# aghasemzadeh/OpenMPL

Hardware: AMD Instinct MI355X
Metric: poses/sec (V=4, J=17, batch=1024 per GPU) fp32 (higher is better)
Workload: dtype f32; 1 GPU; Human3.6M config: V=4 J=17 batch=1024 fp32, CHOSEN flag set, depth 12, DIM 32, heads 8; global_batch=1024, parallelism=single GPU

## Files before the change

### openmpl_amd/csrc/spt_packed.hip

```cpp
#include "spt_pack.hpp"
#include "spt_stage.hpp"

namespace mpl {

constexpr int ATS = 36;
constexpr int HS = 68;
constexpr int KV_F = SJ * SH * SEQ * 4;
constexpr int SPT3_RING_BYTES = (ROWS * XS + 2 * KV_F + ROWS * ATS) * 4;
constexpr int SPT3_LDS_BYTES = 160 * 1024;
constexpr int SPT3_HID_OFF = 3072;
constexpr int SPT3_Q_OFF = 20480;
static_assert(SPT3_HID_OFF + ROWS * HS <= 2 * KV_F + ROWS * ATS, "HID does not fit its alias");
static_assert((SPT3_HID_OFF + ROWS * HS - 2 * KV_F) * 4 <= SPT3_Q_OFF, "HID reaches into the staged qkv weights");
static_assert(SPT3_Q_OFF + 12 * 1024 <= ROWS * ATS * 4, "staged qkv weights do not fit behind HID in ATT");
static_assert(SPT3_RING_BYTES + 8 * 1024 + 2 * SPT3_NPAR * 4 <= SPT3_LDS_BYTES, "spare LDS too small");

typedef float f32x2 __attribute__((ext_vector_type(2)));

__device__ inline float spt_window_scale(float v) {
    if (!(v > 0.f) || !(v < 3.0e38f)) return 1.0f;
    int e;
    (void)frexpf(32768.0f / v, &e);
    e = e - 1 < -100 ? -100 : (e - 1 > 100 ? 100 : e - 1);
    return ldexpf(1.0f, e);
}

__global__ __launch_bounds__(256) void spt_pack_kernel(const float* __restrict__ qkv_w, const float* __restrict__ qkv_b,
                                                        const float* __restrict__ ln1_w, const float* __restrict__ ln1_b,
                                                        const float* __restrict__ proj_w, const float* __restrict__ proj_b,
                                                        const float* __restrict__ fc1_w, const float* __restrict__ fc1_b,
                                                        const float* __restrict__ ln2_w, const float* __restrict__ ln2_b,
                                                        const float* __restrict__ fc2_w, const float* __restrict__ fc2_b,
                                                        char* __restrict__ dst, int fold_q) {
    __shared__ float Wf[8192];
    __shared__ float cn[SPT_NCOL], sw[SPT_NCOL], bnd[SPT_NCOL], scal[2];
    const int tid = threadIdx.x;
    for (int i = tid; i < 8192; i += 256) {
        float w;
        if (i < 3072) w = qkv_w[i] * ln1_w[i & 31];
        else if (i < 4096) w = proj_w[i - 3072];
        else if (i < 6144) w = fc1_w[i - 4096] * ln2_w[i & 31];
        else w = fc2_w[i - 6144];
        Wf[i] = w;
    }
    __syncthreads();
    if (tid < SPT_NCOL) {
        const int n = tid;
        const float *wr, *raw, *beta = nullptr;
        int K = 32;
        float bias;
        if (n < 96) { wr = Wf + n * 32; raw = qkv_w + n * 32; beta = ln1_b; bias = qkv_b[n]; }
        else if (n < 128) { wr = Wf + 3072 + (n - 96) * 32; raw = proj_w + (n - 96) * 32; bias = proj_b[n - 96]; }
        else if (n < 192) { wr = Wf + 4096 + (n - 128) * 32; raw = fc1_w + (n - 128) * 32; beta = ln2_b; bias = fc1_b[n - 128]; }
        else { wr = Wf + 6144 + (n - 192) * 64; raw = fc2_w + (n - 192) * 64; bias = fc2_b[n - 192]; K = 64; }
        float amax = 0.f;
        double ss = 0.0, c = (double)bias;
        for (int k = 0; k < K; ++k) {
            amax = fmaxf(amax, fabsf(wr[k]));
            ss += (double)wr[k] * (double)wr[k];
            if (beta) c += (double)raw[k] * (double)beta[k];
        }
        float s = 1.0f;
        if (amax > 0.f && amax < 3.0e38f) {
            int e;
            (void)frexpf(amax, &e);
            e = 14 - e;
            e = e < -100 ? -100 : (e > 100 ? 100 : e);
            s = ldexpf(1.0f, e);
        }
        cn[n] = (float)c;
        sw[n] = s;
        bnd[n] = beta ? (float)(sqrt(32.0) * sqrt(ss)) + fabsf((float)c) : 0.f;
    }
    __syncthreads();
    if (tid == 0) {
        float batt = 0.f, bhid = 0.f;
        for (int n = 64; n < 96; ++n) batt = fmaxf(batt, bnd[n]);
        for (int n = SPT_C_FC1; n < SPT_C_FC2; ++n) bhid = fmaxf(bhid, bnd[n]);
        scal[0] = spt_window_scale(batt);
        scal[1] = spt_window_scale(bhid);
    }
    __syncthreads();
    float* vec = reinterpret_cast<float*>(dst + SPT_PACK_VEC);
    if (tid < SPT_NCOL) {
        const int n = tid;
        float c = cn[n], sc;
        if (n < 96) sc = 1.0f / (SPT_SA * sw[n]);
        else if (n < 128) sc = 1.0f / (scal[0] * sw[n]);
        else if (n < 192) sc = 1.0f / (SPT_SA * sw[n]);
        else sc = 1.0f / (scal[1] * sw[n]);
        if (n < 32 && fold_q) { c *= SPT_QS; sc *= SPT_QS; }
        vec[n] = c;
        vec[SPT_NCOL + n] = sc;
    }
    if (tid < 8) vec[2 * SPT_NCOL + tid] = tid == 0 ? scal[0] : (tid == 1 ? 0.5f * scal[1] : 0.f);
    sf16x8* frag = reinterpret_cast<sf16x8*>(dst);
    for (int idx = tid; idx < 16 * 64; idx += 256) {
        const int lane = idx & 63, u = idx >> 6, li = lane & 15, kq = lane >> 4;
        const float* src;
        int n;
        if (u < 6) { n = 16 * u + li; src = Wf + n * 32 + 8 * kq; }
        else if (u < 8) { n = 16 * (u - 6) + li; src = Wf + 3072 + n * 32 + 8 * kq; n += SPT_C_PROJ; }
        else if (u < 12) { n = 16 * (u - 8) + li; src = Wf + 4096 + n * 32 + 8 * kq; n += SPT_C_FC1; }
        else { n = 16 * ((u - 12) >> 1) + li; src = Wf + 6144 + n * 64 + 32 * ((u - 12) & 1) + 8 * kq; n += SPT_C_FC2; }
        float x[8];
#pragma unroll
        for (int j = 0; j < 8; ++j) x[j] = src[j] * sw[n];
        sf16x8 hi, lo;
        spt_split2(x, hi, lo);
        frag[(size_t)(u * 2) * 64 + lane] = hi;
        frag[(size_t)(u * 2 + 1) * 64 + lane] = lo;
    }
}

int launch_spt_pack(const mpl_block_weights* bw_host, unsigned short* dst, int fold_q, hipStream_t s) {
    const mpl_block_weights* b = bw_host;
    if (!b || !dst || !b->qkv_w || !b->proj_w || !b->fc1_w || !b->fc2_w || !b->qkv_b || !b->proj_b || !b->fc1_b || !b->fc2_b ||
        !b->ln1_w || !b->ln1_b || !b->ln2_w || !b->ln2_b)
        return MPL_E_INVALID;
    ProfScope prof(MPL_K_PACK, s);
    hipLaunchKernelGGL(spt_pack_kernel, dim3(1), dim3(256), 0, s, b->qkv_w, b->qkv_b, b->ln1_w, b->ln1_b, b->proj_w, b->proj_b, b->fc1_w,
                       b->fc1_b, b->ln2_w, b->ln2_b, b->fc2_w, b->fc2_b, reinterpret_cast<char*>(dst), fold_q);
    return hip_check_launch();
}

size_t spt_pack_bytes() { return SPT_PACK_BYTES; }

template <int SS>
__global__ __launch_bounds__(NTHR, 1) void spt3_kernel(const SptParams p) {
    constexpr int RLIVE = SJ * SS;
    constexpr int MTS = (RLIVE + 15) / 16;
    constexpr int NT = (MTS + 3) / 4;
    extern __shared__ __attribute__((aligned(16))) float smem[];
    float* X = smem;
    float* Kb = smem + ROWS * XS;
    float* Vb = Kb + KV_F;
    float* ATT = Vb + KV_F;
    float* HID = Kb + SPT3_HID_OFF;
    char* S_W = reinterpret_cast<char*>(ATT + ROWS * ATS);
    float* S_PAR = reinterpret_cast<float*>(S_W + 8 * 1024);
    char* R_F1 = reinterpret_cast<char*>(Kb);
    char* R_Q = reinterpret_cast<char*>(ATT) + SPT3_Q_OFF;

    const int tid = threadIdx.x, lane = tid & 63;
    const int wave = __builtin_amdgcn_readfirstlane(tid >> 6);
    const int li = lane & 15, kq = lane >> 4;
    auto phase_sync = [&]() {
        asm volatile("s_waitcnt vmcnt(0)" ::: "memory");
        __syncthreads();
    };
    const int hg = wave & 1, part = wave >> 1;
    const int view = blockIdx.x % p.V;
    const int b0 = (blockIdx.x / p.V) * SS;
    const int sl = li % SS;
    const mpl_spt_set set = p.sets[(p.flags & MPL_F_MULTI_SPT) ? view : 0];
    const float* pose = p.poses[view];
    const float* ray = p.rays[view];
    const float* cen = p.centers[view];

    auto stage_w = [&](char* dst, const unsigned short* pack, int byte_off, int n_pieces) {
        const unsigned l0 = (unsigned)(uintptr_t)(__attribute__((address_space(3))) char*)dst;
        for (int i = wave; i < n_pieces; i += NWAVE)
            ::mpl::dma16(reinterpret_cast<const float*>(reinterpret_cast<const char*>(pack) + byte_off + i * 1024) + lane * 4,
                         l0 + (unsigned)(i * 1024));
    };
    auto load_par = [&](const mpl_block_weights& b) -> float4 {
        if (tid >= SPT3_NPAR / 4) return float4{0.f, 0.f, 0.f, 0.f};
        return ld4(G(reinterpret_cast<const float*>(reinterpret_cast<const char*>(b.qkv_w3) + SPT_PACK_VEC)) + 4 * tid);
    };
    auto store_par = [&](int app_of, const float4& v) {
        if (tid < SPT3_NPAR / 4) st4(S_PAR + (app_of & 1) * SPT3_NPAR + 4 * tid, v);
    };
    mpl_block_weights bw;
    if (p.n_apps > 0) {
        bw = set.blocks[p.sched[0] & 0x7f];
        stage_w(R_Q, bw.qkv_w3, SPT_PACK_QKV, 12);
    }
    const float4 par0 = p.n_apps > 0 ? load_par(bw) : float4{0.f, 0.f, 0.f, 0.f};
    spt_embed<true, SS>(p, set, X, tid, b0, pose, ray, cen, SS, MTS * 16);
    store_par(0, par0);
    phase_sync();

    auto load_w = [&](const char* region, int unit, sf16x8 (&w)[2]) { spt_load_unit(region, unit, lane, w); };
    auto ln_frag = [&](int m, sf16x8& ah, sf16x8& al) {
        const float* xr = X + (m * 16 + li) * XS + 8 * kq;
        spt_ln_split(::mpl::ld4(xr), ::mpl::ld4(xr + 4), ah, al);
    };
    auto raw_frag = [&](const float* rowp, sf16x8& ah, sf16x8& al) {
        const float4 x0 = ::mpl::ld4(rowp), x1 = ::mpl::ld4(rowp + 4);
        const float y[8] = {x0.x, x0.y, x0.z, x0.w, x1.x, x1.y, x1.z, x1.w};
        spt_split2(y, ah, al);
    };

    for (int app = 0; app < p.n_apps; ++app) {
        const bool weighted = (p.sched[app] & 0x80) != 0;
        bw = set.blocks[p.sched[app] & 0x7f];
        const unsigned short* pack = bw.qkv_w3;
        const float* par = S_PAR + (app & 1) * SPT3_NPAR;
        stage_w(S_W, pack, SPT_PACK_PROJ, 4);
        {
            sf16x8 wq[3][2];
            float4 bq[3], sq[3];
#pragma unroll
            for (int c = 0; c < 3; ++c) {
                load_w(R_Q, 2 * c + hg, wq[c]);
                bq[c] = ::mpl::ld4(par + SPT_C_QKV + 32 * c + 16 * hg + 4 * kq);
                sq[c] = ::mpl::ld4(par + SPT_NCOL + SPT_C_QKV + 32 * c + 16 * hg + 4 * kq);
            }
            float4 q[NT];
#pragma unroll
            for (int t = 0; t < NT; ++t) {
                q[t] = float4{0.f, 0.f, 0.f, 0.f};
                if (part + 4 * t < MTS && !(p.abl & 8)) {
                    const int m = part + 4 * t;
                    const int j = (16 * m + li) / SS;
                    const bool live = 16 * m + li < RLIVE;
                    sf16x8 ah, al;
                    ln_frag(m, ah, al);
                    const f32x4 z = {0.f, 0.f, 0.f, 0.f};
                    const f32x4 cq = mfma3(wq[0], ah, al, z), ck = mfma3(wq[1], ah, al, z), cv = mfma3(wq[2], ah, al, z);
                    q[t] = float4{fmaf(cq[0], sq[0].x, bq[0].x), fmaf(cq[1], sq[0].y, bq[0].y), fmaf(cq[2], sq[0].z, bq[0].z),
                                  fmaf(cq[3], sq[0].w, bq[0].w)};
                    const int h = 4 * hg + kq;
                    const float kx = fmaf(ck[0], sq[1].x, bq[1].x), ky = fmaf(ck[1], sq[1].y, bq[1].y);
                    const float kz = fmaf(ck[2], sq[1].z, bq[1].z), kw = fmaf(ck[3], sq[1].w, bq[1].w);
                    if (live && j < SJ - 1) {
                        float* kp = Kb + ((((j >> 1) * 2) * SH + h) * SS + sl) * 4 + (j & 1);
                        kp[0] = kx;
                        kp[2] = ky;
                        kp[SH * SS * 4] = kz;
                        kp[SH * SS * 4 + 2] = kw;
                    } else if (live) {
                        st4(Kb + (SJ - 1) * SH * SS * 4 + (h * SS + sl) * 4, float4{kx, ky, kz, kw});
                    }
                    if (live)
                        st4(Vb + ((j * SH + h) * SS + sl) * 4, float4{fmaf(cv[0], sq[2].x, bq[2].x), fmaf(cv[1], sq[2].y, bq[2].y),
                                                                       fmaf(cv[2], sq[2].z, bq[2].z), fmaf(cv[3], sq[2].w, bq[2].w)});
                }
            }
            phase_sync();
            if (!(p.abl & 1)) {
                const int h = 4 * hg + kq;
                float sc[NT][SJ];
#pragma unroll
                for (int jp = 0; jp < SJ / 2; ++jp) {
                    const float4 k01 = ::mpl::ld4(Kb + (((jp * 2) * SH + h) * SS + sl) * 4);
                    const float4 k23 = ::mpl::ld4(Kb + (((jp * 2 + 1) * SH + h) * SS + sl) * 4);
                    const f32x2 kx = {k01.x, k01.y}, ky = {k01.z, k01.w}, kz = {k23.x, k23.y}, kw = {k23.z, k23.w};
#pragma unroll
                    for (int t = 0; t < NT; ++t) {
                        const f32x2 qx = {q[t].x, q[t].x}, qy = {q[t].y, q[t].y}, qz = {q[t].z, q[t].z}, qw = {q[t].w, q[t].w};
                        f32x2 s2 = qx * kx;
                        s2 = __builtin_elementwise_fma(qy, ky, s2);
                        s2 = __builtin_elementwise_fma(qz, kz, s2);
                        s2 = __builtin_elementwise_fma(qw, kw, s2);
                        sc[t][2 * jp] = s2[0];
                        sc[t][2 * jp + 1] = s2[1];
                    }
                }
                {
                    const float4 k = ::mpl::ld4(Kb + (SJ - 1) * SH * SS * 4 + (h * SS + sl) * 4);
#pragma unroll
                    for (int t = 0; t < NT; ++t)
                        sc[t][SJ - 1] = fmaf(q[t].w, k.w, fmaf(q[t].z, k.z, fmaf(q[t].y, k.y, q[t].x * k.x)));
                }
                const float s_att = par[2 * SPT_NCOL];
                float inv[NT];
#pragma unroll
                for (int t = 0; t < NT; ++t) {
                    float mx = sc[t][0];
#pragma unroll
                    for (int j = 1; j < SJ; ++j) mx = fmaxf(mx, sc[t][j]);
                    float l = 0.f;
#pragma unroll
                    for (int j = 0; j < SJ; ++j) {
                        sc[t][j] = __builtin_amdgcn_exp2f(sc[t][j] - mx);
                        l += sc[t][j];
                    }
                    inv[t] = __builtin_amdgcn_rcpf(l) * s_att;
                    if (weighted) {
                        const int b = b0 + sl, r = 16 * (part + 4 * t) + li;
                        inv[t] *= (b < p.B && r < RLIVE) ? pose[((size_t)b * SJ + r / SS) * 3 + 2] : 0.f;
                    }
                }
                float4 o[NT];
#pragma unroll
                for (int t = 0; t < NT; ++t) o[t] = float4{0.f, 0.f, 0.f, 0.f};
#pragma unroll
                for (int j = 0; j < SJ; ++j) {
                    const float4 v = ::mpl::ld4(Vb + ((j * SH + h) * SS + sl) * 4);
#pragma unroll
                    for (int t = 0; t < NT; ++t) {
                        const float pj = sc[t][j];
                        o[t].x = fmaf(pj, v.x, o[t].x);
                        o[t].y = fmaf(pj, v.y, o[t].y);
                        o[t].z = fmaf(pj, v.z, o[t].z);
                        o[t].w = fmaf(pj, v.w, o[t].w);
                    }
                }
#pragma unroll
                for (int t = 0; t < NT; ++t) {
                    o[t] = float4{o[t].x * inv[t], o[t].y * inv[t], o[t].z * inv[t], o[t].w * inv[t]};
                    if (weighted) {
                        const float big = fmaxf(fmaxf(fabsf(o[t].x), fabsf(o[t].y)), fmaxf(fabsf(o[t].z), fabsf(o[t].w)));
                        if (!(big <= 65000.f)) {
                            const float qn = __builtin_nanf("");
                            o[t] = float4{qn, qn, qn, qn};
                            if (p.err_host) __hip_atomic_fetch_or(p.err_host, 2u, __ATOMIC_RELAXED, __HIP_MEMORY_SCOPE_SYSTEM);
                        }
                    }
                }
#pragma unroll
                for (int t = 0; t < NT; ++t)
                    if (part + 4 * t < MTS) st4(ATT + ((part + 4 * t) * 16 + li) * ATS + 4 * h, o[t]);
            }
        }
        phase_sync();
        {
            stage_w(R_F1, pack, SPT_PACK_FC1, 8);
            sf16x8 wp[2][2];
            float4 bp[2], sp[2];
#pragma unroll
            for (int n = 0; n < 2; ++n) {
                load_w(S_W, n, wp[n]);
                bp[n] = ::mpl::ld4(par + SPT_C_PROJ + 16 * n + 4 * kq);
                sp[n] = ::mpl::ld4(par + SPT_NCOL + SPT_C_PROJ + 16 * n + 4 * kq);
            }
            const int lo = (MTS * 2 * wave) / NWAVE, hi = (MTS * 2 * (wave + 1)) / NWAVE;
            for (int m = lo >> 1; m <= ((hi - 1) >> 1) && !(p.abl & 32); ++m) {
                sf16x8 ah, al;
                raw_frag(ATT + (m * 16 + li) * ATS + 8 * kq, ah, al);
#pragma unroll
                for (int n = 0; n < 2; ++n) {
                    const int u = 2 * m + n;
                    if (u < lo || u >= hi) continue;
                    const f32x4 c = mfma3(wp[n], ah, al, f32x4{0.f, 0.f, 0.f, 0.f});
                    float* xd = X + (m * 16 + li) * XS + 16 * n + 4 * kq;
                    const float4 x = ::mpl::ld4(xd);
                    st4(xd, float4{x.x + fmaf(c[0], sp[n].x, bp[n].x), x.y + fmaf(c[1], sp[n].y, bp[n].y),
                                   x.z + fmaf(c[2], sp[n].z, bp[n].z), x.w + fmaf(c[3], sp[n].w, bp[n].w)});
                }
            }
        }
        phase_sync();
        {
            stage_w(S_W, pack, SPT_PACK_FC2, 8);
            sf16x8 w1[4][2];
            float4 b1[4], s1[4];
#pragma unroll
            for (int n = 0; n < 4; ++n) {
                load_w(R_F1, n, w1[n]);
                b1[n] = ::mpl::ld4(par + SPT_C_FC1 + 16 * n + 4 * kq);
                s1[n] = ::mpl::ld4(par + SPT_NCOL + SPT_C_FC1 + 16 * n + 4 * kq);
            }
            const float hs = par[2 * SPT_NCOL + 1];
            const int lo = (MTS * 4 * wave) / NWAVE, hi = (MTS * 4 * (wave + 1)) / NWAVE;
            for (int m = lo >> 2; m <= ((hi - 1) >> 2) && !(p.abl & 64); ++m) {
                sf16x8 ah, al;
                ln_frag(m, ah, al);
#pragma unroll
                for (int n = 0; n < 4; ++n) {
                    const int u = 4 * m + n;
                    if (u < lo || u >= hi) continue;
                    const f32x4 c = mfma3(w1[n], ah, al, f32x4{0.f, 0.f, 0.f, 0.f});
                    st4(HID + (m * 16 + li) * HS + 16 * n + 4 * kq,
                        float4{gelu_as_scaled(fmaf(c[0], s1[n].x, b1[n].x), hs), gelu_as_scaled(fmaf(c[1], s1[n].y, b1[n].y), hs),
                               gelu_as_scaled(fmaf(c[2], s1[n].z, b1[n].z), hs), gelu_as_scaled(fmaf(c[3], s1[n].w, b1[n].w), hs)});
                }
            }
        }
        phase_sync();
        {
            float4 parn = float4{0.f, 0.f, 0.f, 0.f};
            if (app + 1 < p.n_apps) {
                const mpl_block_weights bn = set.blocks[p.sched[app + 1] & 0x7f];
                stage_w(R_Q, bn.qkv_w3, SPT_PACK_QKV, 12);
                parn = load_par(bn);
            }
            sf16x8 w2[2][2][2];
            float4 b2[2], s2[2];
#pragma unroll
            for (int n = 0; n < 2; ++n) {
                load_w(S_W, 2 * n, w2[n][0]);
                load_w(S_W, 2 * n + 1, w2[n][1]);
                b2[n] = ::mpl::ld4(par + SPT_C_FC2 + 16 * n + 4 * kq);
                s2[n] = ::mpl::ld4(par + SPT_NCOL + SPT_C_FC2 + 16 * n + 4 * kq);
            }
            const int lo = (MTS * 2 * wave) / NWAVE, hi = (MTS * 2 * (wave + 1)) / NWAVE;
            for (int m = lo >> 1; m <= ((hi - 1) >> 1) && !(p.abl & 128); ++m) {
                sf16x8 ah0, al0, ah1, al1;
                raw_frag(HID + (m * 16 + li) * HS + 8 * kq, ah0, al0);
                raw_frag(HID + (m * 16 + li) * HS + 32 + 8 * kq, ah1, al1);
#pragma unroll
                for (int n = 0; n < 2; ++n) {
                    const int u = 2 * m + n;
                    if (u < lo || u >= hi) continue;
                    f32x4 c = mfma3(w2[n][0], ah0, al0, f32x4{0.f, 0.f, 0.f, 0.f});
                    c = mfma3(w2[n][1], ah1, al1, c);
                    float* xd = X + (m * 16 + li) * XS + 16 * n + 4 * kq;
                    const float4 x = ::mpl::ld4(xd);
                    st4(xd, float4{x.x + fmaf(c[0], s2[n].x, b2[n].x), x.y + fmaf(c[1], s2[n].y, b2[n].y),
                                   x.z + fmaf(c[2], s2[n].z, b2[n].z), x.w + fmaf(c[3], s2[n].w, b2[n].w)});
                }
            }
            if (app + 1 < p.n_apps) store_par(app + 1, parn);
        }
        phase_sync();
    }
    spt_epilogue<true, SS>(p, X, tid, view, b0, pose, ray, cen, SS, MTS * 16);
}

template <int SS>
static int launch_spt3(const SptParams& p, int grid, hipStream_t s) {
    if (int rc = kernel_lds_once<spt3_kernel<SS>>(SPT3_LDS_BYTES)) return rc;
    hipLaunchKernelGGL(spt3_kernel<SS>, dim3(grid), dim3(NTHR), SPT3_LDS_BYTES, s, p);
    return hip_check_launch();
}

int launch_spt_packed(const SptParams& p, int ss, int grid, hipStream_t s) {
    switch (ss) {
        case 1: return launch_spt3<1>(p, grid, s);
        case 2: return launch_spt3<2>(p, grid, s);
        case 4: return launch_spt3<4>(p, grid, s);
        case 8: return launch_spt3<8>(p, grid, s);
        case 16: return launch_spt3<16>(p, grid, s);
        default: return MPL_E_INVALID;
    }
}

}
```

### openmpl_amd/csrc/spt_stage.hpp

```cpp
#pragma once
#include "common.hpp"

namespace mpl {

constexpr int SJ = 17;
constexpr int SD = 32;
constexpr int SH = 8;
constexpr int SEQ = 16;
constexpr int ROWS = SEQ * SJ;
constexpr int XS = 36;
constexpr int NTHR = 512;
constexpr int NWAVE = NTHR / 64;
constexpr int SPT_SMALL_SPW = 8;

struct SptParams {
    const float* poses[MPL_MAX_VIEWS];
    const float* rays[MPL_MAX_VIEWS];
    const float* centers[MPL_MAX_VIEWS];
    const mpl_spt_set* sets;
    const float *snorm_w, *snorm_b;
    const float *pos3d_embed, *pos3d_view, *pos3d_lin_w, *pos3d_lin_b;
    const float *ray_w, *ray_b, *cfpt_w, *cfpt_b;
    float* xs;
    int B, V, in_ch, n_apps;
    unsigned flags;
    int c3;
    int spw;
    int abl;
    unsigned* err_host;
    unsigned char sched[MPL_MAX_APPS];
};

int launch_spt_native(const SptParams& p, int form, int grid, hipStream_t s);
int launch_spt_packed(const SptParams& p, int ss, int grid, hipStream_t s);

typedef const __attribute__((address_space(1))) float* gfp;
__device__ __forceinline__ gfp G(const float* p) { return (gfp)p; }
__device__ __forceinline__ float4 ld4(gfp p) {
    typedef float v4 __attribute__((ext_vector_type(4)));
    const v4 t = *reinterpret_cast<const __attribute__((address_space(1))) v4*>(p);
    return make_float4(t.x, t.y, t.z, t.w);
}

template <bool TM, int SS = SEQ>
__device__ __forceinline__ void row_to_sj(int r, int& sq, int& j) {
    if (TM) { j = r / SS; sq = r % SS; }
    else { sq = r / SJ; j = r - sq * SJ; }
}

template <bool TM, int SS = SEQ>
__device__ __forceinline__ void spt_embed(const SptParams& p, const mpl_spt_set& set, float* X, int tid, int b0,
                                          const float* pose, const float* ray, const float* cen, int nseq = SEQ, int nrows = ROWS) {
    for (int idx = tid; idx < nrows * SD; idx += NTHR) {
        const int r = idx >> 5, c = idx & 31;
        int sq, j;
        row_to_sj<TM, SS>(r, sq, j);
        const int b = b0 + sq;
        float x = 0.f;
        if (b < p.B && sq < nseq && j < SJ) {
            const float* in = pose + ((size_t)b * SJ + j) * 3;
            const float* we = set.embed_w + c * p.in_ch;
            x = set.embed_b[c] + we[0] * in[0] + we[1] * in[1];
            if (p.in_ch == 3) x += we[2] * in[2];
            if (p.flags & MPL_F_CONF_ADD) x += set.conf_w[c] * in[2] + set.conf_b[c];
            if (p.flags & MPL_F_CONF_MULT) x *= set.conf_w[c] * in[2] + set.conf_b[c];
            x += set.pos_embed[j * SD + c];
            if (p.flags & MPL_F_POS3D_SPATIAL) {
                if (p.flags & MPL_F_POS3D_LEARN) {
                    x += p.pos3d_embed[j * p.c3 + c];
                } else {
                    const float* rr = ray + ((size_t)b * SJ + j) * 3;
                    const float* cc = cen + (size_t)b * 3;
                    const float vx = rr[0] - cc[0], vy = rr[1] - cc[1], vz = rr[2] - cc[2];
                    const float nrm = fmaxf(sqrtf(vx * vx + vy * vy + vz * vz), 1e-12f);
                    const float* wl = p.pos3d_lin_w + c * 3;
                    x += p.pos3d_lin_b[c] + wl[0] * (vx / nrm) + wl[1] * (vy / nrm) + wl[2] * (vz / nrm);
                }
            }
        }
        X[r * XS + c] = x;
    }
}

template <bool TM, int SS = SEQ>
__device__ __forceinline__ void spt_epilogue(const SptParams& p, const float* X, int tid, int view, int b0, const float* pose,
                                             const float* ray, const float* cen, int nseq = SEQ, int nrows = ROWS) {
    const bool to_rays = (p.flags & MPL_F_POS3D_TO_RAYS) && (p.flags & MPL_F_RAYS_TOKEN);
    const bool ray_tok = !(p.flags & MPL_F_POS3D_TO_RAYS) && (p.flags & MPL_F_RAYS_TOKEN);
    const int cw = to_rays ? 2 * SD : SD;
    const int Df = SJ * SD * ((p.flags & MPL_F_RAYS_TOKEN) ? 2 : 1);
    for (int r = tid; r < nrows; r += NTHR) {
        int sq, j;
        row_to_sj<TM, SS>(r, sq, j);
        const int b = b0 + sq;
        if (b >= p.B || sq >= nseq || j >= SJ) continue;
        const float* xr = X + r * XS;
        float v[SD];
        float s = 0.f;
#pragma unroll
        for (int c = 0; c < SD; c += 4) {
            const float4 t = ld4(xr + c);
            v[c] = t.x; v[c + 1] = t.y; v[c + 2] = t.z; v[c + 3] = t.w;
            s += (t.x + t.y) + (t.z + t.w);
        }
        const float mean = s * (1.0f / 32.0f);
        float ss = 0.f;
#pragma unroll
        for (int c = 0; c < SD; ++c) {
            v[c] -= mean;
            ss = fmaf(v[c], v[c], ss);
        }
        const float rstd = 1.0f / sqrtf(ss * (1.0f / 32.0f) + 1e-6f);
        const float conf = pose[((size_t)b * SJ + j) * 3 + 2];
        float dx = 0.f, dy = 0.f, dz = 0.f, nx = 0.f, ny = 0.f, nz = 0.f;
        const bool need_dir = (p.flags & MPL_F_RAYS_TOKEN) ||
                              (!(p.flags & MPL_F_POS3D_SPATIAL) && !(p.flags & MPL_F_POS3D_LEARN));
        if (need_dir) {
            const float* rr = ray + ((size_t)b * SJ + j) * 3;
            const float* cc = cen + (size_t)b * 3;
            dx = rr[0] - cc[0]; dy = rr[1] - cc[1]; dz = rr[2] - cc[2];
            const float nrm = fmaxf(sqrtf(dx * dx + dy * dy + dz * dz), 1e-12f);
            nx = dx / nrm; ny = dy / nrm; nz = dz / nrm;
        }
        auto pos3d = [=](int c) -> float {
            if (p.flags & MPL_F_POS3D_SPATIAL) return p.pos3d_view[j * p.c3 + c];
            if (p.flags & MPL_F_POS3D_LEARN) return p.pos3d_embed[j * p.c3 + c];
            const float* wl = p.pos3d_lin_w + c * 3;
            return p.pos3d_lin_b[c] + wl[0] * nx + wl[1] * ny + wl[2] * nz;
        };
        auto ray_emb = [=](int c) -> float {
            const float* wr = p.ray_w + c * 3;
            return p.ray_b[c] + wr[0] * dx + wr[1] * dy + wr[2] * dz;
        };
        float* orow = p.xs + ((size_t)b * p.V + view) * Df;
        float* o1 = orow + j * cw;
#pragma unroll
        for (int c = 0; c < SD; c += 4) {
            float t[4];
#pragma unroll
            for (int q = 0; q < 4; ++q) {
                float y = v[c + q] * rstd * p.snorm_w[c + q] + p.snorm_b[c + q];
                if (p.flags & MPL_F_CONF_IN_FPT) y += p.cfpt_w[c + q] * conf + p.cfpt_b[c + q];
                t[q] = y + pos3d(c + q);
            }
            st4(o1 + c, float4{t[0], t[1], t[2], t[3]});
        }
        if (to_rays) {
#pragma unroll
            for (int c = 0; c < SD; c += 4) {
                float t[4];
#pragma unroll
                for (int q = 0; q < 4; ++q) t[q] = ray_emb(c + q) + pos3d(SD + c + q);
                st4(o1 + SD + c, float4{t[0], t[1], t[2], t[3]});
            }
        } else if (ray_tok) {
            float* o2 = orow + (SJ + j) * SD;
#pragma unroll
            for (int c = 0; c < SD; c += 4) st4(o2 + c, float4{ray_emb(c), ray_emb(c + 1), ray_emb(c + 2), ray_emb(c + 3)});
        }
    }
}

}
```

Measured before the change: 889,200 poses/s.

## Template spatial-transformer kernel on wave count and chunk attention queries into groups

```diff
diff --git a/openmpl_amd/csrc/spt_packed.hip b/openmpl_amd/csrc/spt_packed.hip
--- a/openmpl_amd/csrc/spt_packed.hip
+++ b/openmpl_amd/csrc/spt_packed.hip
@@ -126,11 +126,13 @@
 
 size_t spt_pack_bytes() { return SPT_PACK_BYTES; }
 
-template <int SS>
-__global__ __launch_bounds__(NTHR, 1) void spt3_kernel(const SptParams p) {
+template <int SS, int NW, int QG>
+__global__ __launch_bounds__(64 * NW, 1) void spt3_kernel(const SptParams p) {
     constexpr int RLIVE = SJ * SS;
     constexpr int MTS = (RLIVE + 15) / 16;
-    constexpr int NT = (MTS + 3) / 4;
+    constexpr int P = NW / 2;
+    constexpr int NT = (MTS + P - 1) / P;
+    static_assert(NW % 2 == 0 && NW >= 2 && NW <= 16 && QG >= 1, "two head groups per joint class");
     extern __shared__ __attribute__((aligned(16))) float smem[];
     float* X = smem;
     float* Kb = smem + ROWS * XS;
@@ -160,7 +162,7 @@
 
     auto stage_w = [&](char* dst, const unsigned short* pack, int byte_off, int n_pieces) {
         const unsigned l0 = (unsigned)(uintptr_t)(__attribute__((address_space(3))) char*)dst;
-        for (int i = wave; i < n_pieces; i += NWAVE)
+        for (int i = wave; i < n_pieces; i += NW)
             ::mpl::dma16(reinterpret_cast<const float*>(reinterpret_cast<const char*>(pack) + byte_off + i * 1024) + lane * 4,
                          l0 + (unsigned)(i * 1024));
     };
@@ -177,7 +179,7 @@
         stage_w(R_Q, bw.qkv_w3, SPT_PACK_QKV, 12);
     }
     const float4 par0 = p.n_apps > 0 ? load_par(bw) : float4{0.f, 0.f, 0.f, 0.f};
-    spt_embed<true, SS>(p, set, X, tid, b0, pose, ray, cen, SS, MTS * 16);
+    spt_embed<true, SS, 64 * NW>(p, set, X, tid, b0, pose, ray, cen, SS, MTS * 16);
     store_par(0, par0);
     phase_sync();
 
@@ -211,8 +213,8 @@
 #pragma unroll
             for (int t = 0; t < NT; ++t) {
                 q[t] = float4{0.f, 0.f, 0.f, 0.f};
-                if (part + 4 * t < MTS && !(p.abl & 8)) {
-                    const int m = part + 4 * t;
+                if (part + P * t < MTS && !(p.abl & 8)) {
+                    const int m = part + P * t;
                     const int j = (16 * m + li) / SS;
                     const bool live = 16 * m + li < RLIVE;
                     sf16x8 ah, al;
@@ -241,78 +243,90 @@
             phase_sync();
             if (!(p.abl & 1)) {
                 const int h = 4 * hg + kq;
-                float sc[NT][SJ];
-#pragma unroll
-                for (int jp = 0; jp < SJ / 2; ++jp) {
-                    const float4 k01 = ::mpl::ld4(Kb + (((jp * 2) * SH + h) * SS + sl) * 4);
-                    const float4 k23 = ::mpl::ld4(Kb + (((jp * 2 + 1) * SH + h) * SS + sl) * 4);
-                    const f32x2 kx = {k01.x, k01.y}, ky = {k01.z, k01.w}, kz = {k23.x, k23.y}, kw = {k23.z, k23.w};
-#pragma unroll
-                    for (int t = 0; t < NT; ++t) {
-                        const f32x2 qx = {q[t].x, q[t].x}, qy = {q[t].y, q[t].y}, qz = {q[t].z, q[t].z}, qw = {q[t].w, q[t].w};
-                        f32x2 s2 = qx * kx;
-                        s2 = __builtin_elementwise_fma(qy, ky, s2);
-                        s2 = __builtin_elementwise_fma(qz, kz, s2);
-                        s2 = __builtin_elementwise_fma(qw, kw, s2);
-                        sc[t][2 * jp] = s2[0];
-                        sc[t][2 * jp + 1] = s2[1];
-                    }
-                }
-                {
-                    const float4 k = ::mpl::ld4(Kb + (SJ - 1) * SH * SS * 4 + (h * SS + sl) * 4);
-#pragma unroll
-                    for (int t = 0; t < NT; ++t)
-                        sc[t][SJ - 1] = fmaf(q[t].w, k.w, fmaf(q[t].z, k.z, fmaf(q[t].y, k.y, q[t].x * k.x)));
-                }
                 const float s_att = par[2 * SPT_NCOL];
-                float inv[NT];
-#pragma unroll
-                for (int t = 0; t < NT; ++t) {
-                    float mx = sc[t][0];
-#pragma unroll
-                    for (int j = 1; j < SJ; ++j) mx = fmaxf(mx, sc[t][j]);
-                    float l = 0.f;
-#pragma unroll
-                    for (int j = 0; j < SJ; ++j) {
-                        sc[t][j] = __builtin_amdgcn_exp2f(sc[t][j] - mx);
-                        l += sc[t][j];
-                    }
-                    inv[t] = __builtin_amdgcn_rcpf(l) * s_att;
-                    if (weighted) {
-                        const int b = b0 + sl, r = 16 * (part + 4 * t) + li;
-                        inv[t] *= (b < p.B && r < RLIVE) ? pose[((size_t)b * SJ + r / SS) * 3 + 2] : 0.f;
-                    }
-                }
-                float4 o[NT];
-#pragma unroll
-                for (int t = 0; t < NT; ++t) o[t] = float4{0.f, 0.f, 0.f, 0.f};
-#pragma unroll
-                for (int j = 0; j < SJ; ++j) {
-                    const float4 v = ::mpl::ld4(Vb + ((j * SH + h) * SS + sl) * 4);
-#pragma unroll
-                    for (int t = 0; t < NT; ++t) {
-                        const float pj = sc[t][j];
-                        o[t].x = fmaf(pj, v.x, o[t].x);
-                        o[t].y = fmaf(pj, v.y, o[t].y);
-                        o[t].z = fmaf(pj, v.z, o[t].z);
-                        o[t].w = fmaf(pj, v.w, o[t].w);
-                    }
-                }
-#pragma unroll
-                for (int t = 0; t < NT; ++t) {
-                    o[t] = float4{o[t].x * inv[t], o[t].y * inv[t], o[t].z * inv[t], o[t].w * inv[t]};
-                    if (weighted) {
-                        const float big = fmaxf(fmaxf(fabsf(o[t].x), fabsf(o[t].y)), fmaxf(fabsf(o[t].z), fabsf(o[t].w)));
-                        if (!(big <= 65000.f)) {
-                            const float qn = __builtin_nanf("");
-                            o[t] = float4{qn, qn, qn, qn};
-                            if (p.err_host) __hip_atomic_fetch_or(p.err_host, 2u, __ATOMIC_RELAXED, __HIP_MEMORY_SCOPE_SYSTEM);
+#pragma unroll
+                for (int g = 0; g < NT; g += QG) {
+                    if (part + P * g < MTS) {
+                        float sc[QG][SJ];
+#pragma unroll
+                        for (int jp = 0; jp < SJ / 2; ++jp) {
+                            const float4 k01 = ::mpl::ld4(Kb + (((jp * 2) * SH + h) * SS + sl) * 4);
+                            const float4 k23 = ::mpl::ld4(Kb + (((jp * 2 + 1) * SH + h) * SS + sl) * 4);
+                            const f32x2 kx = {k01.x, k01.y}, ky = {k01.z, k01.w}, kz = {k23.x, k23.y}, kw = {k23.z, k23.w};
+#pragma unroll
+                            for (int u = 0; u < QG; ++u) {
+                                if (g + u >= NT) continue;
+                                const float4 qt = q[g + u];
+                                const f32x2 qx = {qt.x, qt.x}, qy = {qt.y, qt.y}, qz = {qt.z, qt.z}, qw = {qt.w, qt.w};
+                                f32x2 s2 = qx * kx;
+                                s2 = __builtin_elementwise_fma(qy, ky, s2);
+                                s2 = __builtin_elementwise_fma(qz, kz, s2);
+                                s2 = __builtin_elementwise_fma(qw, kw, s2);
+                                sc[u][2 * jp] = s2[0];
+                                sc[u][2 * jp + 1] = s2[1];
+                            }
+                        }
+                        {
+                            const float4 k = ::mpl::ld4(Kb + (SJ - 1) * SH * SS * 4 + (h * SS + sl) * 4);
+#pragma unroll
+                            for (int u = 0; u < QG; ++u) {
+                                if (g + u >= NT) continue;
+                                const float4 qt = q[g + u];
+                                sc[u][SJ - 1] = fmaf(qt.w, k.w, fmaf(qt.z, k.z, fmaf(qt.y, k.y, qt.x * k.x)));
+                            }
+                        }
+                        float inv[QG];
+#pragma unroll
+                        for (int u = 0; u < QG; ++u) {
+                            if (g + u >= NT) continue;
+                            float mx = sc[u][0];
+#pragma unroll
+                            for (int j = 1; j < SJ; ++j) mx = fmaxf(mx, sc[u][j]);
+                            float l = 0.f;
+#pragma unroll
+                            for (int j = 0; j < SJ; ++j) {
+                                sc[u][j] = __builtin_amdgcn_exp2f(sc[u][j] - mx);
+                                l += sc[u][j];
+                            }
+                            inv[u] = __builtin_amdgcn_rcpf(l) * s_att;
+                            if (weighted) {
+                                const int b = b0 + sl, r = 16 * (part + P * (g + u)) + li;
+                                inv[u] *= (b < p.B && r < RLIVE) ? pose[((size_t)b * SJ + r / SS) * 3 + 2] : 0.f;
+                            }
+                        }
+                        float4 o[QG];
+#pragma unroll
+                        for (int u = 0; u < QG; ++u) o[u] = float4{0.f, 0.f, 0.f, 0.f};
+#pragma unroll
+                        for (int j = 0; j < SJ; ++j) {
+                            const float4 v = ::mpl::ld4(Vb + ((j * SH + h) * SS + sl) * 4);
+#pragma unroll
+                            for (int u = 0; u < QG; ++u) {
+                                if (g + u >= NT) continue;
+                                const float pj = sc[u][j];
+                                o[u].x = fmaf(pj, v.x, o[u].x);
+                                o[u].y = fmaf(pj, v.y, o[u].y);
+                                o[u].z = fmaf(pj, v.z, o[u].z);
+                                o[u].w = fmaf(pj, v.w, o[u].w);
+                            }
+                        }
+#pragma unroll
+                        for (int u = 0; u < QG; ++u) {
+                            if (g + u >= NT) continue;
+                            o[u] = float4{o[u].x * inv[u], o[u].y * inv[u], o[u].z * inv[u], o[u].w * inv[u]};
+                            if (weighted) {
+                                const float big = fmaxf(fmaxf(fabsf(o[u].x), fabsf(o[u].y)), fmaxf(fabsf(o[u].z), fabsf(o[u].w)));
+                                if (!(big <= 65000.f)) {
+                                    const float qn = __builtin_nanf("");
+                                    o[u] = float4{qn, qn, qn, qn};
+                                    if (p.err_host) __hip_atomic_fetch_or(p.err_host, 2u, __ATOMIC_RELAXED, __HIP_MEMORY_SCOPE_SYSTEM);
+                                }
+                            }
+                            if (part + P * (g + u) < MTS) st4(ATT + ((part + P * (g + u)) * 16 + li) * ATS + 4 * h, o[u]);
                         }
                     }
+                    __builtin_amdgcn_sched_barrier(0);
                 }
-#pragma unroll
-                for (int t = 0; t < NT; ++t)
-                    if (part + 4 * t < MTS) st4(ATT + ((part + 4 * t) * 16 + li) * ATS + 4 * h, o[t]);
             }
         }
         phase_sync();
@@ -326,7 +340,7 @@
                 bp[n] = ::mpl::ld4(par + SPT_C_PROJ + 16 * n + 4 * kq);
                 sp[n] = ::mpl::ld4(par + SPT_NCOL + SPT_C_PROJ + 16 * n + 4 * kq);
             }
-            const int lo = (MTS * 2 * wave) / NWAVE, hi = (MTS * 2 * (wave + 1)) / NWAVE;
+            const int lo = (MTS * 2 * wave) / NW, hi = (MTS * 2 * (wave + 1)) / NW;
             for (int m = lo >> 1; m <= ((hi - 1) >> 1) && !(p.abl & 32); ++m) {
                 sf16x8 ah, al;
                 raw_frag(ATT + (m * 16 + li) * ATS + 8 * kq, ah, al);
@@ -354,7 +368,7 @@
                 s1[n] = ::mpl::ld4(par + SPT_NCOL + SPT_C_FC1 + 16 * n + 4 * kq);
             }
             const float hs = par[2 * SPT_NCOL + 1];
-            const int lo = (MTS * 4 * wave) / NWAVE, hi = (MTS * 4 * (wave + 1)) / NWAVE;
+            const int lo = (MTS * 4 * wave) / NW, hi = (MTS * 4 * (wave + 1)) / NW;
             for (int m = lo >> 2; m <= ((hi - 1) >> 2) && !(p.abl & 64); ++m) {
                 sf16x8 ah, al;
                 ln_frag(m, ah, al);
@@ -386,7 +400,7 @@
                 b2[n] = ::mpl::ld4(par + SPT_C_FC2 + 16 * n + 4 * kq);
                 s2[n] = ::mpl::ld4(par + SPT_NCOL + SPT_C_FC2 + 16 * n + 4 * kq);
             }
-            const int lo = (MTS * 2 * wave) / NWAVE, hi = (MTS * 2 * (wave + 1)) / NWAVE;
+            const int lo = (MTS * 2 * wave) / NW, hi = (MTS * 2 * (wave + 1)) / NW;
             for (int m = lo >> 1; m <= ((hi - 1) >> 1) && !(p.abl & 128); ++m) {
                 sf16x8 ah0, al0, ah1, al1;
                 raw_frag(HID + (m * 16 + li) * HS + 8 * kq, ah0, al0);
@@ -407,13 +421,18 @@
         }
         phase_sync();
     }
-    spt_epilogue<true, SS>(p, X, tid, view, b0, pose, ray, cen, SS, MTS * 16);
-}
+    spt_epilogue<true, SS, 64 * NW>(p, X, tid, view, b0, pose, ray, cen, SS, MTS * 16);
+}
+
+template <int SS> struct spt3_form { static constexpr int NW = 12, QG = 1; };
+template <> struct spt3_form<8> { static constexpr int NW = 8, QG = 2; };
+template <> struct spt3_form<1> { static constexpr int NW = 8, QG = 1; };
 
 template <int SS>
 static int launch_spt3(const SptParams& p, int grid, hipStream_t s) {
-    if (int rc = kernel_lds_once<spt3_kernel<SS>>(SPT3_LDS_BYTES)) return rc;
-    hipLaunchKernelGGL(spt3_kernel<SS>, dim3(grid), dim3(NTHR), SPT3_LDS_BYTES, s, p);
+    constexpr int NW = spt3_form<SS>::NW, QG = spt3_form<SS>::QG;
+    if (int rc = kernel_lds_once<spt3_kernel<SS, NW, QG>>(SPT3_LDS_BYTES)) return rc;
+    hipLaunchKernelGGL((spt3_kernel<SS, NW, QG>), dim3(grid), dim3(64 * NW), SPT3_LDS_BYTES, s, p);
     return hip_check_launch();
 }
 
diff --git a/openmpl_amd/csrc/spt_stage.hpp b/openmpl_amd/csrc/spt_stage.hpp
--- a/openmpl_amd/csrc/spt_stage.hpp
+++ b/openmpl_amd/csrc/spt_stage.hpp
@@ -48,10 +48,10 @@
     else { sq = r / SJ; j = r - sq * SJ; }
 }
 
-template <bool TM, int SS = SEQ>
+template <bool TM, int SS = SEQ, int THREADS = NTHR>
 __device__ __forceinline__ void spt_embed(const SptParams& p, const mpl_spt_set& set, float* X, int tid, int b0,
                                           const float* pose, const float* ray, const float* cen, int nseq = SEQ, int nrows = ROWS) {
-    for (int idx = tid; idx < nrows * SD; idx += NTHR) {
+    for (int idx = tid; idx < nrows * SD; idx += THREADS) {
         const int r = idx >> 5, c = idx & 31;
         int sq, j;
         row_to_sj<TM, SS>(r, sq, j);
@@ -82,14 +82,14 @@
     }
 }
 
-template <bool TM, int SS = SEQ>
+template <bool TM, int SS = SEQ, int THREADS = NTHR>
 __device__ __forceinline__ void spt_epilogue(const SptParams& p, const float* X, int tid, int view, int b0, const float* pose,
                                              const float* ray, const float* cen, int nseq = SEQ, int nrows = ROWS) {
     const bool to_rays = (p.flags & MPL_F_POS3D_TO_RAYS) && (p.flags & MPL_F_RAYS_TOKEN);
     const bool ray_tok = !(p.flags & MPL_F_POS3D_TO_RAYS) && (p.flags & MPL_F_RAYS_TOKEN);
     const int cw = to_rays ? 2 * SD : SD;
     const int Df = SJ * SD * ((p.flags & MPL_F_RAYS_TOKEN) ? 2 : 1);
-    for (int r = tid; r < nrows; r += NTHR) {
+    for (int r = tid; r < nrows; r += THREADS) {
         int sq, j;
         row_to_sj<TM, SS>(r, sq, j);
         const int b = b0 + sq;
```

Measured after the change: 883,800 poses/s. No clear change (-0.6%).
